# Antiparadox/Spartan-BN254

Hardware: AMD Instinct MI355X
Metric: msm_points_per_s (higher is better)
Workload: dtype u32; 1 GPU; synthetic BN254 G1 MSM, 2^20 uniform Fr scalars x distinct bases per GPU, inputs resident in HBM; steps_in_flight=6

## Files before the change

### spartan-bn254_amd/csrc/glv_kernels.cuh

```cuda
#pragma once
#include "msm_kernels.cuh"

namespace sbn {

namespace glv {
constexpr uint64_t A[2] = {0x8211bbeb7d4f1128ull, 0x6f4d8248eeb859fcull};
constexpr uint64_t B = 0x89d3256894d213e3ull;
constexpr uint64_t C[2] = {0x0be4e1541221250bull, 0x6f4d8248eeb859fdull};
constexpr uint64_t G1[3] = {0x5398fd0300ff6565ull, 0x4ccef014a773d2d2ull, 0x2ull};
constexpr uint64_t G2[2] = {0xd91d232ec7e0b3d7ull, 0x2ull};
constexpr uint64_t R[4] = {0x43e1f593f0000001ull, 0x2833e84879b97091ull, 0xb85045b68181585dull, 0x30644e72e131a029ull};
constexpr uint32_t BETA[8] = {0x607cfd48u, 0xe4bd44e5u, 0xbb966e3du, 0xc28f069fu, 0xe0acccb0u, 0x5e6dd9e7u, 0xe131a029u, 0x30644e72u};
}

template <int NA, int NB>
__device__ __forceinline__ void glv_mul(const uint64_t (&a)[NA], const uint64_t (&b)[NB], uint64_t (&out)[NA + NB]) {
#pragma unroll
  for (int i = 0; i < NA + NB; i++) out[i] = 0;
#pragma unroll
  for (int i = 0; i < NA; i++) {
    uint64_t carry = 0;
#pragma unroll
    for (int j = 0; j < NB; j++) {
      const uint64_t lo = a[i] * b[j], hi = __umul64hi(a[i], b[j]);
      uint64_t s = out[i + j] + lo; uint64_t cy = s < lo ? 1 : 0;
      s += carry; cy += s < carry ? 1 : 0;
      out[i + j] = s; carry = hi + cy;
    }
    out[i + NB] = carry;
  }
}
template <int NB>
__device__ __forceinline__ void glv_mul_lo256(const uint64_t (&a)[4], const uint64_t (&b)[NB], uint64_t (&out)[4]) {
#pragma unroll
  for (int i = 0; i < 4; i++) out[i] = 0;
#pragma unroll
  for (int i = 0; i < 4; i++) {
    uint64_t carry = 0;
#pragma unroll
    for (int j = 0; j < NB && i + j < 4; j++) {
      const uint64_t lo = a[i] * b[j], hi = __umul64hi(a[i], b[j]);
      uint64_t s = out[i + j] + lo; uint64_t cy = s < lo ? 1 : 0;
      s += carry; cy += s < carry ? 1 : 0;
      out[i + j] = s; carry = hi + cy;
    }
    if (i + NB < 4) out[i + NB] = carry;
  }
}
__device__ __forceinline__ bool glv_diff_ge_r(const uint64_t (&x)[4], const uint64_t (&y)[4]) {
  uint64_t d[4], borrow = 0;
#pragma unroll
  for (int i = 0; i < 4; i++) { const uint64_t t = x[i] - y[i]; const uint64_t b1 = x[i] < y[i]; d[i] = t - borrow; borrow = b1 | (t < borrow); }
#pragma unroll
  for (int i = 3; i >= 0; i--) { if (d[i] != glv::R[i]) return d[i] > glv::R[i]; }
  return true;
}
__device__ __forceinline__ void u128_mul_lo(uint64_t a0, uint64_t a1, uint64_t b0, uint64_t b1, uint64_t& o0, uint64_t& o1) {
  o0 = a0 * b0; o1 = __umul64hi(a0, b0) + a0 * b1 + a1 * b0;
}
__device__ __forceinline__ void u128_add(uint64_t& x0, uint64_t& x1, uint64_t y0, uint64_t y1) { const uint64_t s = x0 + y0; x1 += y1 + (s < x0 ? 1 : 0); x0 = s; }
__device__ __forceinline__ void u128_sub(uint64_t& x0, uint64_t& x1, uint64_t y0, uint64_t y1) { const uint64_t b = x0 < y0 ? 1 : 0; x0 -= y0; x1 -= y1 + b; }

__device__ __forceinline__ void glv_split(const uint64_t (&k)[4], uint64_t (&k1)[2], uint64_t (&k2)[2]) {
  uint64_t p1[7], p2[6];
  glv_mul<4, 3>(k, glv::G1, p1);
  glv_mul<4, 2>(k, glv::G2, p2);
  uint64_t c1[2] = {p1[4], p1[5]}, c2[1] = {p2[4]};
  {
    uint64_t kc[4], cr[4];
    glv_mul_lo256<2>(k, glv::C, kc);
    const uint64_t c1v[4] = {c1[0], c1[1], 0, 0};
    glv_mul_lo256<4>(c1v, glv::R, cr);
    if (glv_diff_ge_r(kc, cr)) { if (++c1[0] == 0) ++c1[1]; }
  }
  {
    uint64_t kb[4], cr[4];
    const uint64_t bb[1] = {glv::B};
    glv_mul_lo256<1>(k, bb, kb);
    const uint64_t c2v[4] = {c2[0], 0, 0, 0};
    glv_mul_lo256<4>(c2v, glv::R, cr);
    if (glv_diff_ge_r(kb, cr)) ++c2[0];
  }
  uint64_t x0 = k[0], x1 = k[1], t0, t1;
  u128_mul_lo(c1[0], c1[1], glv::A[0], glv::A[1], t0, t1); u128_sub(x0, x1, t0, t1);
  u128_mul_lo(c2[0], 0, glv::B, 0, t0, t1); u128_sub(x0, x1, t0, t1);
  uint64_t y0, y1;
  u128_mul_lo(c1[0], c1[1], glv::B, 0, y0, y1);
  u128_mul_lo(c2[0], 0, glv::C[0], glv::C[1], t0, t1); u128_sub(y0, y1, t0, t1);
  if (y1 >> 63) { u128_add(x0, x1, glv::B, 0); u128_add(y0, y1, glv::C[0], glv::C[1]); }
  k1[0] = x0; k1[1] = x1; k2[0] = y0; k2[1] = y1;
}

__global__ void __launch_bounds__(256) k_glv_split(const uint32_t* __restrict__ scalars, size_t n, uint32_t* __restrict__ out, uint32_t* __restrict__ bad) {
  const size_t t = (size_t)blockIdx.x * blockDim.x + threadIdx.x;
  if (t >= n) return;
  const uint4 a = reinterpret_cast<const uint4*>(scalars + 8 * t)[0], b = reinterpret_cast<const uint4*>(scalars + 8 * t)[1];
  const uint32_t kk[8] = {a.x, a.y, a.z, a.w, b.x, b.y, b.z, b.w};
  uint64_t k1[2] = {0, 0}, k2[2] = {0, 0};
  if (!fe_is_canonical<FrP>(kk)) atomicAdd(bad, 1u);
  else {
    const uint64_t k[4] = {(uint64_t)a.x | ((uint64_t)a.y << 32), (uint64_t)a.z | ((uint64_t)a.w << 32), (uint64_t)b.x | ((uint64_t)b.y << 32), (uint64_t)b.z | ((uint64_t)b.w << 32)};
    glv_split(k, k1, k2);
  }
  uint4* o = reinterpret_cast<uint4*>(out);
  o[t] = make_uint4((uint32_t)k1[0], (uint32_t)(k1[0] >> 32), (uint32_t)k1[1], (uint32_t)(k1[1] >> 32));
  o[n + t] = make_uint4((uint32_t)k2[0], (uint32_t)(k2[0] >> 32), (uint32_t)k2[1], (uint32_t)(k2[1] >> 32));
}

__global__ void __launch_bounds__(256) k_glv_table(const uint32_t* __restrict__ pts, size_t npts, uint32_t* __restrict__ out) {
  const size_t j = (size_t)blockIdx.x * blockDim.x + threadIdx.x;
  if (j >= npts) return;
  const uint4* s = reinterpret_cast<const uint4*>(pts + 16 * j);
  uint4* d0 = reinterpret_cast<uint4*>(out + 16 * j);
  uint4* d1 = reinterpret_cast<uint4*>(out + 16 * (npts + j));
  const uint4 w0 = s[0], w1 = s[1], w2 = s[2], w3 = s[3];
  d0[0] = w0; d0[1] = w1; d0[2] = w2; d0[3] = w3;
  const Fq beta = fe_to_mont(fe_unpack<FqP>(glv::BETA));
  const Fq x = fe_load<FqP>(pts + 16 * j);
  fe_store<FqP>(out + 16 * (npts + j), fe_mul(x, beta));
  d1[2] = w2; d1[3] = w3;
}

}
```

### spartan-bn254_amd/csrc/sort2_kernels.cuh

```cuda
#pragma once
#include "msm_kernels.cuh"
#include <utility>

namespace sbn {

struct S2Geom {
  size_t n;
  int c, W, P;
  int lo_log;
  int K;
  size_t half, gap;
};

template <int C, int SW = 8> struct S2Shape {
  static constexpr int BITS = SW == 8 ? 254 : 127;
  static constexpr int W0 = (BITS + C - 1) / C;
  static constexpr int W = W0 + ((BITS - (W0 - 1) * C) > C - 1 ? 1 : 0);
};
typedef uint32_t s2_u32x8 __attribute__((ext_vector_type(8)));
template <int C, int w> __device__ __forceinline__ int s2_digit(const s2_u32x8 k, uint32_t& carry) {
  constexpr int bit = w * C, limb = bit >> 5, sh = bit & 31;
  uint64_t x = 0;
  if constexpr (limb < 8) x = k[limb];
  if constexpr (limb + 1 < 8) x |= (uint64_t)k[limb + 1] << 32;
  const uint32_t raw = (uint32_t)(x >> sh) & ((1u << C) - 1u);
  const uint32_t v = raw + carry;
  if (v >= (1u << (C - 1))) { carry = 1; return (int)v - (1 << C); }
  carry = 0;
  return (int)v;
}
template <int SW = 8> __device__ __forceinline__ s2_u32x8 s2_load_scalar(const uint32_t* __restrict__ scalars, size_t t) {
  const uint4* p = reinterpret_cast<const uint4*>(scalars + (size_t)SW * t);
  const uint4 a = p[0], b = SW == 8 ? p[1] : make_uint4(0u, 0u, 0u, 0u);
  s2_u32x8 k; k[0] = a.x; k[1] = a.y; k[2] = a.z; k[3] = a.w; k[4] = b.x; k[5] = b.y; k[6] = b.z; k[7] = b.w;
  return k;
}
__device__ __forceinline__ bool s2_is_canonical(const s2_u32x8 k) { uint32_t kk[8]; for (int i = 0; i < 8; i++) kk[i] = k[i]; return fe_is_canonical<FrP>(kk); }

extern __shared__ uint32_t s2_lds[];

template <int C, int... Ws>
__device__ __forceinline__ void s2_count_scalar(const s2_u32x8 kk, int P, int lo_log, std::integer_sequence<int, Ws...>) {
  uint32_t carry = 0;
  auto one = [&](auto wc) {
    constexpr int w = decltype(wc)::value;
    const int d = s2_digit<C, w>(kk, carry);
    if (d != 0) atomicAdd(&s2_lds[w * P + (((d < 0 ? -d : d) - 1) >> lo_log)], 1u);
  };
  (one(std::integral_constant<int, Ws>{}), ...);
}
template <int C, int SPT, int SW = 8>
__global__ void __launch_bounds__(1024) k_s2_count(const uint32_t* __restrict__ scalars, S2Geom g, uint32_t* __restrict__ cntA, uint32_t* __restrict__ bad) {
  constexpr int W = S2Shape<C, SW>::W; constexpr int CH = 1024 * SPT;
  const int k = blockIdx.x, P = g.P;
  for (int j = threadIdx.x; j < W * P; j += 1024) s2_lds[j] = 0;
  __syncthreads();
  for (int i = 0; i < SPT; i++) {
    const size_t t = (size_t)k * CH + (size_t)i * 1024 + threadIdx.x;
    if (t >= g.n) break;
    const s2_u32x8 kk = s2_load_scalar<SW>(scalars, t);
    if (SW == 8 && !s2_is_canonical(kk)) atomicAdd(bad, 1u);
    s2_count_scalar<C>(kk, P, g.lo_log, std::make_integer_sequence<int, W>{});
  }
  __syncthreads();
  for (int j = threadIdx.x; j < W * P; j += 1024) cntA[(size_t)j * g.K + k] = s2_lds[j];
}

__device__ __forceinline__ uint32_t s2_block_scan(uint32_t v, uint32_t* tmp , uint32_t* total) {
  const int lane = threadIdx.x & 63, wv = threadIdx.x >> 6, nw = (blockDim.x + 63) >> 6;
  uint32_t inc = v;
#pragma unroll
  for (int d = 1; d < 64; d <<= 1) { const uint32_t o = __shfl_up(inc, d); if (lane >= d) inc += o; }
  if (lane == 63) tmp[wv] = inc;
  __syncthreads();
  if (threadIdx.x == 0) { uint32_t run = 0; for (int i = 0; i < nw; i++) { const uint32_t x = tmp[i]; tmp[i] = run; run += x; } tmp[16] = run; }
  __syncthreads();
  const uint32_t r = inc - v + tmp[wv];
  *total = tmp[16];
  __syncthreads();
  return r;
}
__global__ void __launch_bounds__(256) k_s2_prefix_k(uint32_t* __restrict__ cntA, int K, uint32_t* __restrict__ part_cnt) {
  __shared__ uint32_t tmp[17];
  uint32_t* row = cntA + (size_t)blockIdx.x * K;
  const int per = (K + 255) / 256, b0 = threadIdx.x * per;
  uint32_t sum = 0;
  for (int i = 0; i < per; i++) if (b0 + i < K) sum += row[b0 + i];
  uint32_t total; uint32_t run = s2_block_scan(sum, tmp, &total);
  for (int i = 0; i < per; i++) if (b0 + i < K) { const uint32_t v = row[b0 + i]; row[b0 + i] = run; run += v; }
  if (threadIdx.x == 0) part_cnt[blockIdx.x] = total;
}
__global__ void __launch_bounds__(1024) k_s2_prefix_hi(const uint32_t* __restrict__ part_cnt, int W, int P, uint32_t* __restrict__ part_off, uint32_t* __restrict__ sc_off) {
  __shared__ uint32_t tmp[17];
  __shared__ uint32_t wstart[32];
  const int n = W * P, per = (n + 1023) / 1024, i0 = (int)threadIdx.x * per, i1 = (i0 + per < n) ? i0 + per : n;
  uint32_t sv = 0, sk = 0;
  for (int i = i0; i < i1; i++) { const uint32_t v = part_cnt[i]; sv += v; sk += (v + S2_SUB - 1) / S2_SUB; }
  uint32_t tv, tk;
  uint32_t rv = s2_block_scan(sv, tmp, &tv), rk = s2_block_scan(sk, tmp, &tk);
  for (int i = i0; i < i1; i++) { const uint32_t v = part_cnt[i]; part_off[i] = rv; sc_off[i] = rk; rv += v; rk += (v + S2_SUB - 1) / S2_SUB; }
  if (threadIdx.x == 0) sc_off[(size_t)n] = tk;
  __syncthreads();
  if ((int)threadIdx.x < W) wstart[threadIdx.x] = part_off[(size_t)threadIdx.x * P];
  __syncthreads();
  for (int i = i0; i < i1; i++) part_off[i] -= wstart[i / P];
}

__host__ __device__ inline size_t s2_scatter_lds_bytes(int P, int spt = S2_SPT) { return ((size_t)3 * P + 32) * 4 + (size_t)1024 * spt * 8; }
struct S2ScatterArgs {
  const uint32_t* cntA; const uint32_t* part_off; uint32_t* tmp_idx; uint16_t* tmp_lo;
  size_t n, half, gap; int P, K, k, lo_log;
};
template <int C, int w, int SPT>
__device__ __forceinline__ void s2_scatter_window(const s2_u32x8 (&kk)[SPT], uint32_t (&carry)[SPT], const S2ScatterArgs& a) {
  constexpr int CH = 1024 * SPT;
  const int P = a.P, tid = threadIdx.x;
  uint32_t* cnt = s2_lds; uint32_t* base = cnt + P; uint32_t* gdelta = base + P; uint32_t* tmp = gdelta + P;
  uint32_t* stage_idx = tmp + 32;
  uint16_t* stage_lo = reinterpret_cast<uint16_t*>(stage_idx + CH); uint16_t* stage_hi = stage_lo + CH;
  for (int j = tid; j < P; j += 1024) cnt[j] = 0;
  __syncthreads();
  int d[SPT]; uint32_t rank[SPT];
#pragma unroll
  for (int i = 0; i < SPT; i++) {
    const int dd = s2_digit<C, w>(kk[i], carry[i]);
    d[i] = dd; rank[i] = 0;
    if (dd != 0) rank[i] = atomicAdd(&cnt[((dd < 0 ? -dd : dd) - 1) >> a.lo_log], 1u);
  }
  __syncthreads();
  uint32_t total;
  {
    const uint32_t v = tid < P ? cnt[tid] : 0;
    const uint32_t r = s2_block_scan(v, tmp, &total);
    if (tid < P) { base[tid] = r; gdelta[tid] = a.part_off[(size_t)w * P + tid] + a.cntA[((size_t)w * P + tid) * a.K + a.k] - r; }
  }
  __syncthreads();
  const size_t t0 = (size_t)a.k * CH + tid;
#pragma unroll
  for (int i = 0; i < SPT; i++) {
    if (d[i] == 0) continue;
    const uint32_t b = (uint32_t)((d[i] < 0 ? -d[i] : d[i]) - 1), hi = b >> a.lo_log;
    const uint32_t pos = base[hi] + rank[i];
    size_t e = t0 + (size_t)i * 1024;
    if (a.gap && e >= a.half) e += a.gap;
    stage_idx[pos] = (uint32_t)e | (d[i] < 0 ? 0x80000000u : 0u);
    stage_lo[pos] = (uint16_t)(b & ((1u << a.lo_log) - 1u)); stage_hi[pos] = (uint16_t)hi;
  }
  __syncthreads();
  uint32_t* oi = a.tmp_idx + (size_t)w * a.n; uint16_t* ol = a.tmp_lo + (size_t)w * a.n;
  for (uint32_t j = tid; j < total; j += 1024) {
    const uint32_t pos = j + gdelta[stage_hi[j]];
    oi[pos] = stage_idx[j]; ol[pos] = stage_lo[j];
  }
  __syncthreads();
}
template <int C, int SPT, int... Ws>
__device__ __forceinline__ void s2_scatter_windows(const s2_u32x8 (&kk)[SPT], uint32_t (&carry)[SPT], const S2ScatterArgs& a, std::integer_sequence<int, Ws...>) {
  (s2_scatter_window<C, Ws, SPT>(kk, carry, a), ...);
}
template <int C, int SPT, int SW = 8>
__global__ void __launch_bounds__(1024) k_s2_scatter(const uint32_t* __restrict__ scalars, S2Geom g, const uint32_t* __restrict__ cntA ,
                                                     const uint32_t* __restrict__ part_off, uint32_t* __restrict__ tmp_idx, uint16_t* __restrict__ tmp_lo) {
  S2ScatterArgs a; a.cntA = cntA; a.part_off = part_off; a.tmp_idx = tmp_idx; a.tmp_lo = tmp_lo; a.n = g.n; a.P = g.P; a.K = g.K; a.k = blockIdx.x; a.lo_log = g.lo_log;
  a.half = g.half; a.gap = SW == 8 ? 0 : g.gap;
  s2_u32x8 kk[SPT]; uint32_t carry[SPT];
#pragma unroll
  for (int i = 0; i < SPT; i++) {
    const size_t t = (size_t)blockIdx.x * (1024 * SPT) + (size_t)i * 1024 + threadIdx.x;
    carry[i] = 0;
    kk[i] = t < g.n ? s2_load_scalar<SW>(scalars, t) : (s2_u32x8)(0u);
  }
  s2_scatter_windows<C, SPT>(kk, carry, a, std::make_integer_sequence<int, S2Shape<C, SW>::W>{});
}

__device__ __forceinline__ bool s2_decode(const S2Geom& g, const uint32_t* __restrict__ sc_off, int& q, uint32_t& sidx, uint32_t& k2) {
  const uint32_t Lid = blockIdx.x, xcd = Lid & 7u, slot = Lid >> 3;
  sidx = (slot >> 4) * 128u + xcd * 16u + (slot & 15u);
  const int WP = g.W * g.P;
  if (sidx >= sc_off[WP]) return false;
  int lo = 0, hi = WP;
  while (hi - lo > 1) { const int mid = (lo + hi) >> 1; if (sc_off[mid] <= sidx) lo = mid; else hi = mid; }
  q = lo; k2 = sidx - sc_off[q];
  return true;
}
__host__ __device__ inline uint32_t s2_level2_blocks(size_t max_subchunks) { return (uint32_t)(((max_subchunks + 127) / 128) * 128); }
__device__ __forceinline__ void s2_range(const S2Geom& g, const uint32_t* __restrict__ part_off, const uint32_t* __restrict__ part_cnt, int q, uint32_t k2, size_t& e0, size_t& e1) {
  const uint32_t start = part_off[q], cn = part_cnt[q];
  uint32_t a = k2 * S2_SUB, b = a + S2_SUB; if (a > cn) a = cn; if (b > cn) b = cn;
  const size_t w = (size_t)(q / g.P);
  e0 = w * g.n + start + a; e1 = w * g.n + start + b;
}
__global__ void __launch_bounds__(1024) k_s2_hist(const uint16_t* __restrict__ tmp_lo, S2Geom g, const uint32_t* __restrict__ part_off, const uint32_t* __restrict__ part_cnt, const uint32_t* __restrict__ sc_off, uint32_t* __restrict__ blockhist) {
  __shared__ uint32_t h[S2_LO_MAX];
  int q; uint32_t sidx, k2; if (!s2_decode(g, sc_off, q, sidx, k2)) return;
  const int LO = 1 << g.lo_log;
  for (int j = threadIdx.x; j < LO; j += 1024) h[j] = 0;
  __syncthreads();
  size_t e0, e1; s2_range(g, part_off, part_cnt, q, k2, e0, e1);
  for (size_t e = e0 + threadIdx.x; e < e1; e += 1024) atomicAdd(&h[tmp_lo[e]], 1u);
  __syncthreads();
  uint32_t* o = blockhist + (size_t)sidx * LO;
  for (int j = threadIdx.x; j < LO; j += 1024) o[j] = h[j];
}
__global__ void __launch_bounds__(1024) k_s2_prefix2(uint32_t* __restrict__ blockhist, S2Geom g, const uint32_t* __restrict__ part_off, const uint32_t* __restrict__ sc_off, uint32_t* __restrict__ hist, uint32_t* __restrict__ offs) {
  __shared__ uint32_t tmp[17];
  const int q = blockIdx.x, LO = 1 << g.lo_log, w = q / g.P, hi = q - w * g.P;
  const uint32_t s0 = sc_off[q], nk = sc_off[q + 1] - s0;
  const int j0 = 2 * threadIdx.x;
  uint32_t r0 = 0, r1 = 0;
  if (j0 < LO) {
    uint2* col = reinterpret_cast<uint2*>(blockhist + (size_t)s0 * LO + j0);
    for (uint32_t k = 0; k < nk; k++) { uint2* pq = col + (size_t)k * (LO / 2); const uint2 v = *pq; *pq = make_uint2(r0, r1); r0 += v.x; r1 += v.y; }
  }
  uint32_t total; const uint32_t r = s2_block_scan(r0 + r1, tmp, &total);
  if (j0 < LO) {
    const size_t b = ((size_t)w * g.P + hi) * LO + j0;
    hist[b] = r0; hist[b + 1] = r1;
    offs[b] = part_off[q] + r; offs[b + 1] = part_off[q] + r + r0;
  }
}
constexpr int S2_EPT = 8;
__host__ __device__ inline size_t s2_place_lds_bytes(int lo_log) { return ((size_t)3 * ((size_t)1 << lo_log) + 32) * 4 + (size_t)1024 * S2_EPT * 6; }
__global__ void __launch_bounds__(1024) k_s2_place(const uint16_t* __restrict__ tmp_lo, const uint32_t* __restrict__ tmp_idx, S2Geom g, const uint32_t* __restrict__ part_off, const uint32_t* __restrict__ part_cnt,
                                                   const uint32_t* __restrict__ sc_off, const uint32_t* __restrict__ blockhist ,
                                                   const uint32_t* __restrict__ offs, uint32_t* __restrict__ sorted, size_t estride) {
  constexpr uint32_t T = 1024 * S2_EPT;
  int q; uint32_t sidx, k2; if (!s2_decode(g, sc_off, q, sidx, k2)) return;
  const int LO = 1 << g.lo_log, tid = threadIdx.x;
  uint32_t* cnt = s2_lds; uint32_t* base = cnt + LO; uint32_t* cur = base + LO; uint32_t* tmp = cur + LO;
  uint32_t* stage_idx = tmp + 32; uint16_t* stage_lo = reinterpret_cast<uint16_t*>(stage_idx + T);
  const int w = q / g.P, hi = q - w * g.P;
  const size_t nb = (size_t)g.P << g.lo_log;
  const uint32_t* b0 = blockhist + (size_t)sidx * LO;
  const uint32_t* of = offs + (size_t)w * nb + ((size_t)hi << g.lo_log);
  for (int j = tid; j < LO; j += 1024) { cur[j] = of[j] + b0[j]; cnt[j] = 0; }
  __syncthreads();
  size_t e0, e1; s2_range(g, part_off, part_cnt, q, k2, e0, e1);
  uint32_t* out = sorted + (size_t)w * estride;
  for (size_t tile = e0; tile < e1; tile += T) {
    uint32_t lo[S2_EPT], idx[S2_EPT], rank[S2_EPT];
#pragma unroll
    for (int i = 0; i < S2_EPT; i++) {
      const size_t e = tile + (size_t)i * 1024 + tid;
      lo[i] = 0xffffffffu;
      if (e < e1) { lo[i] = tmp_lo[e]; idx[i] = tmp_idx[e]; rank[i] = atomicAdd(&cnt[lo[i]], 1u); }
    }
    __syncthreads();
    uint32_t total;
    {
      const int j0 = 2 * tid, j1 = 2 * tid + 1;
      const uint32_t v0 = j0 < LO ? cnt[j0] : 0, v1 = j1 < LO ? cnt[j1] : 0;
      const uint32_t r = s2_block_scan(v0 + v1, tmp, &total);
      if (j0 < LO) base[j0] = r;
      if (j1 < LO) base[j1] = r + v0;
    }
    __syncthreads();
#pragma unroll
    for (int i = 0; i < S2_EPT; i++) {
      if (lo[i] == 0xffffffffu) continue;
      const uint32_t pos = base[lo[i]] + rank[i];
      stage_idx[pos] = idx[i]; stage_lo[pos] = (uint16_t)lo[i];
    }
    __syncthreads();
    for (uint32_t j = tid; j < total; j += 1024) {
      const uint32_t l = stage_lo[j];
      out[cur[l] + (j - base[l])] = stage_idx[j];
    }
    __syncthreads();
    for (int j = tid; j < LO; j += 1024) { cur[j] += cnt[j]; cnt[j] = 0; }
    __syncthreads();
  }
}

}
```

Measured before the change: 779.9 million points/s.

## Rewrite GLV split in signed 28-bit limbs; vectorize sort histogram and scatter loops

The GLV scalar decomposition moves from 64-bit schoolbook multiplies with carry chains to signed 28-bit limb column accumulation in int64, using precomputed negated constants so subtractions fold into the accumulation. This is meant to avoid the costly 64-bit high-multiply and carry handling on the GPU. The sort histogram kernel now reads eight 16-bit digits per 128-bit load, and the scatter loop is unrolled to a fixed S2_EPT trip count. A probe harness for testing the split kernel is also added. The new limb arithmetic adds correctness risk in the floor and correction steps.

Measured after the change: 783.1 million points/s (median of 6 runs). About the same (+0.4%).

```diff
diff --git a/spartan-bn254_amd/csrc/glv_kernels.cuh b/spartan-bn254_amd/csrc/glv_kernels.cuh
--- a/spartan-bn254_amd/csrc/glv_kernels.cuh
+++ b/spartan-bn254_amd/csrc/glv_kernels.cuh
@@ -13,80 +13,103 @@
 constexpr uint32_t BETA[8] = {0x607cfd48u, 0xe4bd44e5u, 0xbb966e3du, 0xc28f069fu, 0xe0acccb0u, 0x5e6dd9e7u, 0xe131a029u, 0x30644e72u};
 }
 
-template <int NA, int NB>
-__device__ __forceinline__ void glv_mul(const uint64_t (&a)[NA], const uint64_t (&b)[NB], uint64_t (&out)[NA + NB]) {
-#pragma unroll
-  for (int i = 0; i < NA + NB; i++) out[i] = 0;
+#if defined(__HIP_DEVICE_COMPILE__)
+#define GLV_PIN(x) asm volatile("" ::"v"(x))
+#define GLV_OPAQUE(x) asm volatile("" : "+v"(x))
+#else
+#define GLV_PIN(x)
+#define GLV_OPAQUE(x)
+#endif
+constexpr int GLV_LB = 28;
+constexpr uint32_t GLV_LM = (1u << GLV_LB) - 1u;
+template <int N> struct GlvLimbs { int32_t v[N]; };
+template <int N> constexpr GlvLimbs<N> glv_limbs(const uint64_t* x, int nx, int lsh, int sign) {
+  GlvLimbs<N> r{};
+  for (int i = 0; i < N; i++) {
+    uint32_t v = 0;
+    for (int t = 0; t < GLV_LB; t++) { const int p = GLV_LB * i + t - lsh; if (p >= 0 && p < 64 * nx && ((x[p >> 6] >> (p & 63)) & 1)) v |= 1u << t; }
+    r.v[i] = sign * (int32_t)v;
+  }
+  return r;
+}
+namespace glv {
+constexpr uint64_t B1[1] = {B};
+constexpr GlvLimbs<6> G1L = glv_limbs<6>(G1, 3, 24, 1);
+constexpr GlvLimbs<4> G2L = glv_limbs<4>(G2, 2, 24, 1);
+constexpr GlvLimbs<5> CL = glv_limbs<5>(C, 2, 0, 1), CN = glv_limbs<5>(C, 2, 0, -1), AN = glv_limbs<5>(A, 2, 0, -1);
+constexpr GlvLimbs<3> BL = glv_limbs<3>(B1, 1, 0, 1), BN = glv_limbs<3>(B1, 1, 0, -1);
+constexpr GlvLimbs<10> RN = glv_limbs<10>(R, 4, 0, -1);
+constexpr GlvLimbs<1> ONE = {{1}};
+}
+template <int NA, int NB> __device__ __forceinline__ void glv_col(int64_t& acc, const uint32_t (&a)[NA], const GlvLimbs<NB>& b, int col) {
 #pragma unroll
   for (int i = 0; i < NA; i++) {
-    uint64_t carry = 0;
-#pragma unroll
-    for (int j = 0; j < NB; j++) {
-      const uint64_t lo = a[i] * b[j], hi = __umul64hi(a[i], b[j]);
-      uint64_t s = out[i + j] + lo; uint64_t cy = s < lo ? 1 : 0;
-      s += carry; cy += s < carry ? 1 : 0;
-      out[i + j] = s; carry = hi + cy;
-    }
-    out[i + NB] = carry;
+    const int j = col - i;
+    if (j < 0 || j >= NB) continue;
+    acc += (int64_t)(int32_t)a[i] * (int64_t)b.v[j];
+    GLV_PIN(acc);
   }
 }
-template <int NB>
-__device__ __forceinline__ void glv_mul_lo256(const uint64_t (&a)[4], const uint64_t (&b)[NB], uint64_t (&out)[4]) {
+template <int NG, int NC> __device__ __forceinline__ void glv_floor(const uint32_t (&kl)[10], const GlvLimbs<NG>& g, uint32_t (&c)[NC]) {
+  int64_t acc = 0;
 #pragma unroll
-  for (int i = 0; i < 4; i++) out[i] = 0;
-#pragma unroll
-  for (int i = 0; i < 4; i++) {
-    uint64_t carry = 0;
-#pragma unroll
-    for (int j = 0; j < NB && i + j < 4; j++) {
-      const uint64_t lo = a[i] * b[j], hi = __umul64hi(a[i], b[j]);
-      uint64_t s = out[i + j] + lo; uint64_t cy = s < lo ? 1 : 0;
-      s += carry; cy += s < carry ? 1 : 0;
-      out[i + j] = s; carry = hi + cy;
-    }
-    if (i + NB < 4) out[i + NB] = carry;
+  for (int col = 0; col < 10 + NC; col++) {
+    glv_col<10, NG>(acc, kl, g, col);
+    if (col >= 10) c[col - 10] = (uint32_t)acc & GLV_LM;
+    acc >>= GLV_LB;
   }
 }
-__device__ __forceinline__ bool glv_diff_ge_r(const uint64_t (&x)[4], const uint64_t (&y)[4]) {
-  uint64_t d[4], borrow = 0;
+template <int NX, int NC> __device__ __forceinline__ void glv_correct(const uint32_t (&kl)[10], const GlvLimbs<NX>& x, uint32_t (&c)[NC]) {
+  uint32_t cp[NC];
 #pragma unroll
-  for (int i = 0; i < 4; i++) { const uint64_t t = x[i] - y[i]; const uint64_t b1 = x[i] < y[i]; d[i] = t - borrow; borrow = b1 | (t < borrow); }
+  for (int i = 0; i < NC; i++) cp[i] = c[i];
+  cp[0] += 1;
+  int64_t acc = 0;
+  uint32_t top = 0;
 #pragma unroll
-  for (int i = 3; i >= 0; i--) { if (d[i] != glv::R[i]) return d[i] > glv::R[i]; }
-  return true;
+  for (int col = 0; col < 10; col++) {
+    glv_col<10, NX>(acc, kl, x, col);
+    glv_col<NC, 10>(acc, cp, glv::RN, col);
+    top = (uint32_t)acc;
+    acc >>= GLV_LB;
+  }
+  c[0] += 1u - ((top >> (GLV_LB - 1)) & 1u);
 }
-__device__ __forceinline__ void u128_mul_lo(uint64_t a0, uint64_t a1, uint64_t b0, uint64_t b1, uint64_t& o0, uint64_t& o1) {
-  o0 = a0 * b0; o1 = __umul64hi(a0, b0) + a0 * b1 + a1 * b0;
+__device__ __forceinline__ void glv_pack128(const uint32_t (&l)[5], uint64_t& o0, uint64_t& o1) {
+  o0 = (uint64_t)l[0] | ((uint64_t)l[1] << 28) | ((uint64_t)l[2] << 56);
+  o1 = ((uint64_t)l[2] >> 8) | ((uint64_t)l[3] << 20) | ((uint64_t)l[4] << 48);
 }
 __device__ __forceinline__ void u128_add(uint64_t& x0, uint64_t& x1, uint64_t y0, uint64_t y1) { const uint64_t s = x0 + y0; x1 += y1 + (s < x0 ? 1 : 0); x0 = s; }
-__device__ __forceinline__ void u128_sub(uint64_t& x0, uint64_t& x1, uint64_t y0, uint64_t y1) { const uint64_t b = x0 < y0 ? 1 : 0; x0 -= y0; x1 -= y1 + b; }
 
 __device__ __forceinline__ void glv_split(const uint64_t (&k)[4], uint64_t (&k1)[2], uint64_t (&k2)[2]) {
-  uint64_t p1[7], p2[6];
-  glv_mul<4, 3>(k, glv::G1, p1);
-  glv_mul<4, 2>(k, glv::G2, p2);
-  uint64_t c1[2] = {p1[4], p1[5]}, c2[1] = {p2[4]};
-  {
-    uint64_t kc[4], cr[4];
-    glv_mul_lo256<2>(k, glv::C, kc);
-    const uint64_t c1v[4] = {c1[0], c1[1], 0, 0};
-    glv_mul_lo256<4>(c1v, glv::R, cr);
-    if (glv_diff_ge_r(kc, cr)) { if (++c1[0] == 0) ++c1[1]; }
+  uint32_t kl[10];
+#pragma unroll
+  for (int i = 0; i < 10; i++) {
+    const int bit = GLV_LB * i, limb = bit >> 6, sh = bit & 63;
+    uint64_t x = k[limb] >> sh;
+    if (sh > 64 - GLV_LB && limb + 1 < 4) x |= k[limb + 1] << (64 - sh);
+    kl[i] = (uint32_t)x & GLV_LM;
   }
-  {
-    uint64_t kb[4], cr[4];
-    const uint64_t bb[1] = {glv::B};
-    glv_mul_lo256<1>(k, bb, kb);
-    const uint64_t c2v[4] = {c2[0], 0, 0, 0};
-    glv_mul_lo256<4>(c2v, glv::R, cr);
-    if (glv_diff_ge_r(kb, cr)) ++c2[0];
+  GLV_OPAQUE(kl[9]);
+  uint32_t c1[5], c2[3];
+  glv_floor<6, 5>(kl, glv::G1L, c1);
+  glv_floor<4, 3>(kl, glv::G2L, c2);
+  glv_correct<5, 5>(kl, glv::CL, c1);
+  glv_correct<3, 3>(kl, glv::BL, c2);
+  uint32_t xl[5], yl[5];
+  int64_t ax = 0, ay = 0;
+#pragma unroll
+  for (int col = 0; col < 5; col++) {
+    glv_col<10, 1>(ax, kl, glv::ONE, col);
+    glv_col<5, 5>(ax, c1, glv::AN, col);
+    glv_col<3, 3>(ax, c2, glv::BN, col);
+    xl[col] = (uint32_t)ax & GLV_LM; ax >>= GLV_LB;
+    glv_col<5, 3>(ay, c1, glv::BL, col);
+    glv_col<3, 5>(ay, c2, glv::CN, col);
+    yl[col] = (uint32_t)ay & GLV_LM; ay >>= GLV_LB;
   }
-  uint64_t x0 = k[0], x1 = k[1], t0, t1;
-  u128_mul_lo(c1[0], c1[1], glv::A[0], glv::A[1], t0, t1); u128_sub(x0, x1, t0, t1);
-  u128_mul_lo(c2[0], 0, glv::B, 0, t0, t1); u128_sub(x0, x1, t0, t1);
-  uint64_t y0, y1;
-  u128_mul_lo(c1[0], c1[1], glv::B, 0, y0, y1);
-  u128_mul_lo(c2[0], 0, glv::C[0], glv::C[1], t0, t1); u128_sub(y0, y1, t0, t1);
+  uint64_t x0, x1, y0, y1;
+  glv_pack128(xl, x0, x1); glv_pack128(yl, y0, y1);
   if (y1 >> 63) { u128_add(x0, x1, glv::B, 0); u128_add(y0, y1, glv::C[0], glv::C[1]); }
   k1[0] = x0; k1[1] = x1; k2[0] = y0; k2[1] = y1;
 }
diff --git a/spartan-bn254_amd/csrc/sort2_kernels.cuh b/spartan-bn254_amd/csrc/sort2_kernels.cuh
--- a/spartan-bn254_amd/csrc/sort2_kernels.cuh
+++ b/spartan-bn254_amd/csrc/sort2_kernels.cuh
@@ -197,7 +197,15 @@
   for (int j = threadIdx.x; j < LO; j += 1024) h[j] = 0;
   __syncthreads();
   size_t e0, e1; s2_range(g, part_off, part_cnt, q, k2, e0, e1);
-  for (size_t e = e0 + threadIdx.x; e < e1; e += 1024) atomicAdd(&h[tmp_lo[e]], 1u);
+  size_t a0 = (e0 + 7) & ~(size_t)7; if (a0 > e1) a0 = e1;
+  const size_t a1 = a0 + ((e1 - a0) & ~(size_t)7);
+  if (e0 + threadIdx.x < a0) atomicAdd(&h[tmp_lo[e0 + threadIdx.x]], 1u);
+  if (a1 + threadIdx.x < e1) atomicAdd(&h[tmp_lo[a1 + threadIdx.x]], 1u);
+  for (size_t e = a0 + (size_t)8 * threadIdx.x; e < a1; e += 8 * 1024) {
+    const uint4 v = *reinterpret_cast<const uint4*>(tmp_lo + e);
+    atomicAdd(&h[v.x & 0xffffu], 1u); atomicAdd(&h[v.x >> 16], 1u); atomicAdd(&h[v.y & 0xffffu], 1u); atomicAdd(&h[v.y >> 16], 1u);
+    atomicAdd(&h[v.z & 0xffffu], 1u); atomicAdd(&h[v.z >> 16], 1u); atomicAdd(&h[v.w & 0xffffu], 1u); atomicAdd(&h[v.w >> 16], 1u);
+  }
   __syncthreads();
   uint32_t* o = blockhist + (size_t)sidx * LO;
   for (int j = threadIdx.x; j < LO; j += 1024) o[j] = h[j];
@@ -262,9 +270,13 @@
       stage_idx[pos] = idx[i]; stage_lo[pos] = (uint16_t)lo[i];
     }
     __syncthreads();
-    for (uint32_t j = tid; j < total; j += 1024) {
-      const uint32_t l = stage_lo[j];
-      out[cur[l] + (j - base[l])] = stage_idx[j];
+#pragma unroll
+    for (int i = 0; i < S2_EPT; i++) {
+      const uint32_t j = (uint32_t)i * 1024u + tid;
+      if (j < total) {
+        const uint32_t l = stage_lo[j];
+        out[cur[l] + (j - base[l])] = stage_idx[j];
+      }
     }
     __syncthreads();
     for (int j = tid; j < LO; j += 1024) { cur[j] += cnt[j]; cnt[j] = 0; }
diff --git a/spartan-bn254_amd/harness/glv_probe.hip b/spartan-bn254_amd/harness/glv_probe.hip
--- /dev/null
+++ b/spartan-bn254_amd/harness/glv_probe.hip
@@ -0,0 +1,34 @@
+#include <hip/hip_runtime.h>
+#include <stdint.h>
+#include <stdio.h>
+
+#include "../csrc/glv_kernels.cuh"
+
+using namespace sbn;
+
+#define PROBE_CHECK(x)                                                                                      \
+  do {                                                                                                      \
+    const hipError_t e_ = (x);                                                                              \
+    if (e_ != hipSuccess) { snprintf(err, errlen, "%s: %s", #x, hipGetErrorString(e_)); rc = -1; goto done; } \
+  } while (0)
+
+extern "C" int glv_probe_split(const void* scalars, size_t n, void* halves, uint32_t* bad, char* err, size_t errlen) {
+  int rc = 0;
+  uint32_t *d_in = nullptr, *d_out = nullptr, *d_bad = nullptr;
+  if (n == 0) return 0;
+  PROBE_CHECK(hipMalloc(&d_in, n * 32));
+  PROBE_CHECK(hipMalloc(&d_out, n * 32));
+  PROBE_CHECK(hipMalloc(&d_bad, 4));
+  PROBE_CHECK(hipMemcpy(d_in, scalars, n * 32, hipMemcpyHostToDevice));
+  PROBE_CHECK(hipMemset(d_bad, 0, 4));
+  hipLaunchKernelGGL(k_glv_split, dim3((unsigned)((n + 255) / 256)), dim3(256), 0, 0, (const uint32_t*)d_in, n, d_out, d_bad);
+  PROBE_CHECK(hipGetLastError());
+  PROBE_CHECK(hipDeviceSynchronize());
+  PROBE_CHECK(hipMemcpy(halves, d_out, n * 32, hipMemcpyDeviceToHost));
+  PROBE_CHECK(hipMemcpy(bad, d_bad, 4, hipMemcpyDeviceToHost));
+done:
+  if (d_in) (void)hipFree(d_in);
+  if (d_out) (void)hipFree(d_out);
+  if (d_bad) (void)hipFree(d_bad);
+  return rc;
+}
```
